# staple/spark-agd

Measured on NVIDIA H100. Metric: AGD examples/sec (rows x applySmooth passes / s), logistic 10M x 1024 dense fp32, higher is better.
Workload: dtype f64

## Files before the change

spark-agd_b200/csrc/k1_tc.cu:

```cuda
#include <cuda.h>
#include <cuda_bf16.h>
#include <cuda_runtime.h>
#include <stdint.h>

#include "agd_common.cuh"
#include "k1_device.cuh"

namespace agd {

namespace {

constexpr int kKR = 16;
constexpr int kRegsConsumer = 64, kRegsAux = 56, kRegsMma = 168;
constexpr int kBlockBytes = kKR * 128;
constexpr int kBBytes = 1024;
constexpr int kScaleOff = 768;

__device__ __forceinline__ uint32_t smem_u32(const void *p) { return (uint32_t)__cvta_generic_to_shared(p); }
__device__ __forceinline__ void mbar_init(uint32_t bar, uint32_t count) {
  asm volatile("mbarrier.init.shared::cta.b64 [%0], %1;" ::"r"(bar), "r"(count));
}
__device__ __forceinline__ void mbar_expect_tx(uint32_t bar, uint32_t bytes) {
  asm volatile("mbarrier.arrive.expect_tx.shared::cta.b64 _, [%0], %1;" ::"r"(bar), "r"(bytes) : "memory");
}
__device__ __forceinline__ void mbar_arrive(uint32_t bar) {
  asm volatile("mbarrier.arrive.shared::cta.b64 _, [%0];" ::"r"(bar) : "memory");
}
__device__ __forceinline__ void mbar_wait(uint32_t bar, uint32_t parity) {
  asm volatile(
      "{\n\t.reg .pred p;\n\t"
      "WAIT_LOOP:\n\t"
      "mbarrier.try_wait.parity.shared::cta.b64 p, [%0], %1;\n\t"
      "@p bra WAIT_DONE;\n\t"
      "bra WAIT_LOOP;\n\t"
      "WAIT_DONE:\n\t}" ::"r"(bar),
      "r"(parity)
      : "memory");
}
__device__ __forceinline__ void named_arrive(int id, int count) {
  asm volatile("bar.arrive %0, %1;" ::"r"(id), "r"(count) : "memory");
}
__device__ __forceinline__ void named_sync(int id, int count) {
  asm volatile("bar.sync %0, %1;" ::"r"(id), "r"(count) : "memory");
}
__device__ __forceinline__ void tma_bulk_g2s(uint32_t dst, const void *src, uint32_t bytes, uint32_t bar) {
  asm volatile("cp.async.bulk.shared::cluster.global.mbarrier::complete_tx::bytes [%0], [%1], %2, [%3];" ::"r"(dst),
               "l"(src), "r"(bytes), "r"(bar)
               : "memory");
}
__device__ __forceinline__ void tma_tile_2d(uint32_t dst, const CUtensorMap *map, int c0, int c1, uint32_t bar) {
  asm volatile("cp.async.bulk.tensor.2d.shared::cluster.global.mbarrier::complete_tx::bytes [%0], [%1, {%2, %3}], [%4];" ::"r"(dst),
               "l"(map), "r"(c0), "r"(c1), "r"(bar)
               : "memory");
}
__device__ __forceinline__ void tma_tile_3d(uint32_t dst, const CUtensorMap *map, int c0, int c1, int c2, uint32_t bar) {
  asm volatile("cp.async.bulk.tensor.3d.shared::cluster.global.mbarrier::complete_tx::bytes [%0], [%1, {%2, %3, %4}], [%5];" ::"r"(dst),
               "l"(map), "r"(c0), "r"(c1), "r"(c2), "r"(bar)
               : "memory");
}
__device__ __forceinline__ uint64_t gmma_desc(uint32_t addr, uint32_t lbo, uint32_t sbo, uint64_t layout) {
  return (uint64_t)((addr & 0x3FFFF) >> 4) | ((uint64_t)(lbo >> 4) << 16) | ((uint64_t)(sbo >> 4) << 32) | (layout << 62);
}
__device__ __forceinline__ void wgmma_fence() { asm volatile("wgmma.fence.sync.aligned;" ::: "memory"); }
__device__ __forceinline__ void wgmma_commit() { asm volatile("wgmma.commit_group.sync.aligned;" ::: "memory"); }
template <int N>
__device__ __forceinline__ void wgmma_wait() { asm volatile("wgmma.wait_group.sync.aligned %0;" ::"n"(N) : "memory"); }
template <int N>
__device__ __forceinline__ void wgmma_bf16(float (&d)[N / 2], uint64_t adesc, uint64_t bdesc);
template <>
__device__ __forceinline__ void wgmma_bf16<16>(float (&d)[8], uint64_t adesc, uint64_t bdesc) {
  asm volatile("{ .reg .pred p; setp.ne.b32 p, 0, 0;\n\t"
               "wgmma.mma_async.sync.aligned.m64n16k16.f32.bf16.bf16 {%0,%1,%2,%3,%4,%5,%6,%7}, %8, %9, p, 1, 1, 1, 0; }"
               : "+f"(d[0]), "+f"(d[1]), "+f"(d[2]), "+f"(d[3]), "+f"(d[4]), "+f"(d[5]), "+f"(d[6]), "+f"(d[7])
               : "l"(adesc), "l"(bdesc)
               : "memory");
}
template <>
__device__ __forceinline__ void wgmma_bf16<24>(float (&d)[12], uint64_t adesc, uint64_t bdesc) {
  asm volatile("{ .reg .pred p; setp.ne.b32 p, 0, 0;\n\t"
               "wgmma.mma_async.sync.aligned.m64n24k16.f32.bf16.bf16 {%0,%1,%2,%3,%4,%5,%6,%7,%8,%9,%10,%11}, %12, %13, p, 1, 1, 1, 0; }"
               : "+f"(d[0]), "+f"(d[1]), "+f"(d[2]), "+f"(d[3]), "+f"(d[4]), "+f"(d[5]), "+f"(d[6]), "+f"(d[7]),
                 "+f"(d[8]), "+f"(d[9]), "+f"(d[10]), "+f"(d[11])
               : "l"(adesc), "l"(bdesc)
               : "memory");
}

template <int N, bool TWO>
__device__ __forceinline__ void mma_accumulate(const float (&e)[2][N / 2], int hb, int hs, const double (&sc)[2], double &g,
                                               double *g2) {
  float v[6];
#pragma unroll
  for (int t = 0; t < (TWO ? 6 : 3); ++t) {
    const int i = t == 0 ? 0 : t == 1 ? 1 : t == 2 ? 4 : t == 3 ? 5 : t == 4 ? 8 : 9;
    const float x0 = hs ? e[0][i + 2] : e[0][i], x1 = hs ? e[1][i + 2] : e[1][i];
    v[t] = hb ? x1 : x0;
  }
  g += (((double)v[0] + (double)v[1]) + (double)v[2]) * sc[0];
  if (TWO) *g2 += (((double)v[3] + (double)v[4]) + (double)v[5]) * sc[1];
}
__device__ __forceinline__ double pow2i(int k) { return __longlong_as_double((long long)(k + 1023) << 52); }
__device__ __forceinline__ void mma_release(uint32_t empty_bar, int lane) {
  __syncwarp();
  if (lane == 0) mbar_arrive(empty_bar);
}

struct TcLayout {
  uint32_t ring_off, w_off, b2_off, partial_off, bars_off, g2_off, total;
};
__host__ __device__ inline TcLayout tc_layout(int ring_groups, int group_bytes, int d, bool two_gradient) {
  TcLayout L;
  L.ring_off = 0;
  L.w_off = (uint32_t)ring_groups * group_bytes;
  L.b2_off = L.w_off + (uint32_t)d * 8;
  L.partial_off = L.b2_off + 2 * kBBytes;
  L.bars_off = L.partial_off + 2 * kKR * 16 * 8;
  L.g2_off = L.bars_off + (2 * (uint32_t)ring_groups + 8) * 8;
  L.total = L.g2_off + (two_gradient ? (uint32_t)d * 8 : 0u);
  return L;
}

struct TcArgs {
  const double *labels;
  const double *w;
  const double *w2;
  double *slabs;
  long long rows;
  int d, kind, slab_stride;
  unsigned long long sample_seed, sample_thresh;
  long long row_base;
  int gb;
  int ngt;
  int ring_groups;
  int one_copy;
  int diag;
};

__host__ __device__ constexpr int tc_consumers(int rpt) { return rpt == 4 ? 256 : 512; }
__device__ __forceinline__ unsigned long long ffma2(unsigned long long a, unsigned long long b, unsigned long long c) {
  const float x = __fmaf_rn(__uint_as_float((uint32_t)a), __uint_as_float((uint32_t)b), __uint_as_float((uint32_t)c));
  const float y = __fmaf_rn(__uint_as_float((uint32_t)(a >> 32)), __uint_as_float((uint32_t)(b >> 32)),
                            __uint_as_float((uint32_t)(c >> 32)));
  return ((unsigned long long)__float_as_uint(y) << 32) | __float_as_uint(x);
}
__device__ __forceinline__ unsigned long long pack2(uint32_t lo, uint32_t hi) {
  unsigned long long d;
  asm("mov.b64 %0, {%1, %2};" : "=l"(d) : "r"(lo), "r"(hi));
  return d;
}

template <int RPT, bool F32, int DUAL = 0>
__global__ void __launch_bounds__(tc_consumers(RPT) + 256, 1)
k1_tc_kernel(const __grid_constant__ CUtensorMap tmap, const __grid_constant__ CUtensorMap tmap3, const TcArgs a,
             const long long ntiles) {
  constexpr int kConsumers = tc_consumers(RPT);
  constexpr int kThreads = kConsumers + 256;
  constexpr int kN = DUAL == 2 ? 24 : 16;
  constexpr int kCW = kConsumers / 32;
  constexpr bool kRepartition = RPT != 4;
  extern __shared__ __align__(1024) unsigned char smem[];
  const int group_bytes = a.gb * kBlockBytes;
  const TcLayout L = tc_layout(a.ring_groups, group_bytes, a.d, DUAL == 2);
  double *w_s = reinterpret_cast<double *>(smem + L.w_off);
  unsigned char *b2 = smem + L.b2_off;
  double *partial = reinterpret_cast<double *>(smem + L.partial_off);
  const uint32_t bars = smem_u32(smem + L.bars_off);
  const int RG = a.ring_groups;
  const uint32_t wbar = bars + 16u * RG, b2_full = wbar + 8, b2_empty = b2_full + 16;
  const int tid = threadIdx.x, warp = tid >> 5, lane = tid & 31;
  const long long my_tiles = (ntiles - blockIdx.x + gridDim.x - 1) / gridDim.x;
  const int npairs = a.d / 128;
  double *slab = a.slabs + (size_t)blockIdx.x * a.slab_stride;

  if (tid == 0) {
    for (int g = 0; g < RG; ++g) {
      mbar_init(bars + 8u * g, 1);
      mbar_init(bars + 8u * (RG + g), 4);
    }
    mbar_init(wbar, 1);
    mbar_init(b2_full, 1); mbar_init(b2_full + 8, 1);
    mbar_init(b2_empty, 4); mbar_init(b2_empty + 8, 4);
    asm volatile("fence.mbarrier_init.release.cluster;" ::: "memory");
  }
  for (int i = tid; i < 2 * kBBytes / 4; i += kThreads) reinterpret_cast<uint32_t *>(b2)[i] = 0u;
  asm volatile("fence.proxy.async.shared::cta;" ::: "memory");
  __syncthreads();

  if (warp >= kCW && warp < kCW + 4) {
   if (kRepartition) asm volatile("setmaxnreg.dec.sync.aligned.u32 %0;" ::"n"(kRegsAux));
   if (warp == kCW) {
    if (lane == 0) {
      mbar_expect_tx(wbar, (uint32_t)a.d * 8u);
      tma_bulk_g2s(smem_u32(w_s), a.w, (uint32_t)a.d * 8u, wbar);
      int slot = -1;
      uint32_t epar = 0;
      bool wrapped = false;
      for (long long k = 0; k < my_tiles; ++k) {
        const long long row0 = (blockIdx.x + k * (long long)gridDim.x) * kKR;
        for (int gi = 0; gi < a.ngt; ++gi) {
          if (++slot == RG) { slot = 0; if (wrapped) epar ^= 1u; wrapped = true; }
          if (wrapped) mbar_wait(bars + 8u * (RG + slot), epar);
          const uint32_t full = bars + 8u * slot;
          mbar_expect_tx(full, (uint32_t)group_bytes);
          if (a.one_copy) {
            tma_tile_3d(smem_u32(smem + (size_t)slot * group_bytes), &tmap3, 0, (int)row0, gi * a.gb, full);
          } else {
            for (int b = 0; b < a.gb; ++b)
              tma_tile_2d(smem_u32(smem + (size_t)slot * group_bytes + b * kBlockBytes), &tmap, (gi * a.gb + b) * 64, (int)row0, full);
          }
        }
      }
    }
   } else if (warp == kCW + 2) {
    double lossacc = 0.0, cntacc = 0.0;
    double ynext = 0.0;
    const int srow = lane & 15;
    const bool second = DUAL && lane >= kKR;
    if (lane < kKR || DUAL) {
      const long long r = (long long)blockIdx.x * kKR + srow;
      if (r < a.rows) ynext = a.labels[r];
    }
    const double *partial2 = partial + 2 * kKR * 2;
    for (long long k = 0; k < my_tiles; ++k) {
      const int bb = (int)(k & 1);
      const long long tile = blockIdx.x + k * (long long)gridDim.x;
      const long long left = a.rows - tile * kKR;
      const int rv = left < kKR ? (int)left : kKR;
      const double ylab = ynext;
      if (lane < kKR || DUAL) {
        const long long r = (tile + gridDim.x) * kKR + srow;
        if (r < a.rows) ynext = a.labels[r];
      }
      named_sync(1 + bb, kConsumers + 32);
      double mult = 0.0;
      bool nonfinite = false;
      if (lane < kKR || second) {
        double m;
        if (RPT) {
          const double *pp = second ? partial2 : partial;
          m = pp[(bb * kKR + srow) * 2] + pp[(bb * kKR + srow) * 2 + 1];
        } else {
          const double *pp = partial + (bb * kKR + lane) * 16;
          m = (((pp[0] + pp[1]) + (pp[2] + pp[3])) + ((pp[4] + pp[5]) + (pp[6] + pp[7]))) +
              (((pp[8] + pp[9]) + (pp[10] + pp[11])) + ((pp[12] + pp[13]) + (pp[14] + pp[15])));
        }
        nonfinite = (lane < kKR || DUAL == 2) && srow < rv && !isfinite(m);
        double mu, loss;
        loss_eval(a.kind, m, ylab, mu, loss);
        if (srow < rv && row_selected(a.sample_seed, a.sample_thresh, a.row_base + tile * kKR + srow)) {
          mult = mu; lossacc += loss; cntacc += 1.0;
        }
      }
      named_arrive(3 + bb, kConsumers + 32);
      const uint32_t hw = (uint32_t)__double2hiint(mult) & 0x7fffffffu;
      const uint32_t hwf = hw | (nonfinite ? 0x80000000u : 0u);
      uint32_t top = __reduce_max_sync(0xffffffffu, lane < kKR ? hwf : 0u), top2 = 0u;
      if (DUAL == 2) top2 = __reduce_max_sync(0xffffffffu, lane < kKR ? 0u : hwf);
      if ((top | top2) >> 31) {
        top = __reduce_max_sync(0xffffffffu, lane < kKR ? hw : 0u);
        if (DUAL == 2) top2 = __reduce_max_sync(0xffffffffu, lane < kKR ? 0u : hw);
        const uint32_t fl = __ballot_sync(0xffffffffu, nonfinite && mult == 0.0);
        const uint32_t zero_rows = DUAL == 2 ? (fl & (fl >> 16) & 0xffffu) : fl;
        const int slot0 = (int)((k * a.ngt) % RG);
#pragma unroll 1
        for (uint32_t rows = zero_rows; rows; rows &= rows - 1u) {
          const int zr = __ffs(rows) - 1;
          int sl = slot0;
#pragma unroll 1
          for (int gi = 0; gi < a.ngt; ++gi) {
#pragma unroll 1
            for (int c = lane; c < a.gb * 8; c += 32)
              *reinterpret_cast<uint4 *>(smem + sl * group_bytes + (c >> 3) * kBlockBytes + zr * 128 + (c & 7) * 16) =
                  make_uint4(0u, 0u, 0u, 0u);
            if (++sl == RG) sl = 0;
          }
        }
      }
      uint32_t E = top >> 20;
      if (DUAL == 2 && second) E = top2 >> 20;
      const int s = E == 0x7ffu ? 0 : E == 0u ? -1022 : E == 0x7feu ? 1023 : (int)E - 1022;
      const int ns = -s;
      const double ms = (mult * pow2i(ns >> 1)) * pow2i(ns - (ns >> 1));
      if (k >= 2) mbar_wait(b2_empty + 8u * bb, (uint32_t)(((k >> 1) - 1) & 1));
      if (srow == 0 && (lane < kKR || (DUAL == 2 && second))) {
        reinterpret_cast<double *>(b2 + bb * kBBytes + kScaleOff)[second ? 1 : 0] = pow2i(s);
      }
      if (lane < kKR || (DUAL == 2 && second)) {
        const __nv_bfloat16 hi = __double2bfloat16(ms);
        const double r1 = ms - (double)__bfloat162float(hi);
        const __nv_bfloat16 mid = __double2bfloat16(r1);
        const double r2 = r1 - (double)__bfloat162float(mid);
        const __nv_bfloat16 lo = __double2bfloat16(r2);
        const int n0 = second ? 9 : 0, n1 = second ? 16 : 1, n2 = second ? 17 : 8;
        unsigned char *base = b2 + bb * kBBytes + (srow / 8) * 128 + (srow % 8) * 2;
#pragma unroll
        for (int t = 0; t < 4; ++t) {
          const int c0 = n0 + 2 * t, c1 = n1 + 2 * t, c2 = n2 + 2 * t;
          *reinterpret_cast<__nv_bfloat16 *>(base + (c0 / 8) * 256 + (c0 % 8) * 16) = hi;
          *reinterpret_cast<__nv_bfloat16 *>(base + (c1 / 8) * 256 + (c1 % 8) * 16) = mid;
          *reinterpret_cast<__nv_bfloat16 *>(base + (c2 / 8) * 256 + (c2 % 8) * 16) = lo;
        }
      }
      asm volatile("fence.proxy.async.shared::cta;" ::: "memory");
      __syncwarp();
      if (lane == 0) mbar_arrive(b2_full + 8u * bb);
    }
    for (int off = DUAL ? 8 : 16; off >= 1; off >>= 1) {
      lossacc += __shfl_xor_sync(0xffffffffu, lossacc, off);
      cntacc += __shfl_xor_sync(0xffffffffu, cntacc, off);
    }
    if (lane == 0) { slab[a.d] = lossacc; slab[a.d + 1] = cntacc; if (!DUAL) { slab[a.d + 2] = 0.0; slab[a.d + 3] = 0.0; } }
    if (DUAL && lane == kKR) {
      slab[a.d + 2] = lossacc; slab[a.d + 3] = cntacc;
      if (DUAL == 2) {
        double *slab2 = slab + a.d + 4;
        slab2[a.d] = lossacc; slab2[a.d + 1] = cntacc; slab2[a.d + 2] = 0.0; slab2[a.d + 3] = 0.0;
      }
    }
   }
  } else if (warp >= kCW + 4) {
    if (kRepartition) asm volatile("setmaxnreg.inc.sync.aligned.u32 %0;" ::"n"(kRegsMma));
    const int mw = warp - (kCW + 4);
    const int q = lane >> 2, j = lane & 3;
    const int hb = j >> 1, hs = j & 1;
    const int fo = 64 * hb + 16 * mw + q + 8 * hs;
    double gacc[32];
#pragma unroll
    for (int p = 0; p < 32; ++p) gacc[p] = 0.0;
    double *g2 = reinterpret_cast<double *>(smem + L.g2_off);
    if (DUAL == 2)
      for (int p = 0; p < npairs; ++p) g2[128 * p + fo] = 0.0;
    const int hp = a.gb / 2;
    int slot = -1;
    uint32_t par = 1;
    float acc[2][kN / 2];
    for (long long k = 0; k < my_tiles; ++k) {
      const int bb = (int)(k & 1);
      mbar_wait(b2_full + 8u * bb, (uint32_t)((k >> 1) & 1));
      const uint64_t bdesc = gmma_desc(smem_u32(b2 + bb * kBBytes), 128, 256, 0);
      const double *scs = reinterpret_cast<const double *>(b2 + bb * kBBytes + kScaleOff);
      const double sc[2] = {scs[0], DUAL == 2 ? scs[1] : 1.0};
#pragma unroll
      for (int p = 0; p < 32; ++p) {
        if (p < npairs) {
          const int pg = p % hp;
          if (pg == 0) {
            if (++slot == RG) slot = 0;
            if (slot == 0) par ^= 1u;
            mbar_wait(bars + 8u * slot, par);
          }
          const uint32_t a0 = smem_u32(smem + (size_t)slot * group_bytes + (2 * pg) * kBlockBytes);
          wgmma_fence();
          if (a.diag != 101) {
            wgmma_bf16<kN>(acc[0], gmma_desc(a0, kBlockBytes, 1024, 1), bdesc);
            wgmma_bf16<kN>(acc[1], gmma_desc(a0 + kBlockBytes, kBlockBytes, 1024, 1), bdesc);
          }
          wgmma_commit();
          wgmma_wait<0>();
          mma_accumulate<kN, DUAL == 2>(acc, hb, hs, sc, gacc[p], g2 + 128 * p + fo);
          if (pg == hp - 1) mma_release(bars + 8u * (RG + slot), lane);
        }
      }
      __syncwarp();
      if (lane == 0) mbar_arrive(b2_empty + 8u * bb);
    }
#pragma unroll
    for (int p = 0; p < 32; ++p)
      if (p < npairs) {
        slab[128 * p + fo] = gacc[p];
        if (DUAL == 2) slab[a.d + 4 + 128 * p + fo] = g2[128 * p + fo];
      }
  } else {
    if (kRepartition) asm volatile("setmaxnreg.dec.sync.aligned.u32 %0;" ::"n"(kRegsConsumer));
    if constexpr (RPT == 0) {
      const int r = lane & 15, hsel = lane >> 4;
      mbar_wait(wbar, 0);
      int slot = -1;
      uint32_t par = 1;
      const int npairs = a.gb * 4;
      uint32_t x_off[2];
      int w_off[2];
      bool act[2];
#pragma unroll
      for (int j = 0; j < 2; ++j) {
        const int c = 2 * (warp + 16 * j) + hsel;
        act[j] = warp + 16 * j < npairs;
        x_off[j] = (uint32_t)((c >> 3) * kBlockBytes + r * 128 + (((c & 7) ^ (r & 7)) << 4));
        w_off[j] = c * 8;
      }
      for (long long k = 0; k < my_tiles; ++k) {
        const int bb = (int)(k & 1);
        double pa[2] = {0.0, 0.0}, pb[2] = {0.0, 0.0};
        const double *wp = w_s;
        for (int gi = 0; gi < a.ngt; ++gi) {
          if (++slot == RG) slot = 0;
          if (slot == 0) par ^= 1u;
          mbar_wait(bars + 8u * slot, par);
          if (a.diag != 100) {
            const unsigned char *gbase = smem + (uint32_t)slot * (uint32_t)group_bytes;
#pragma unroll
            for (int j = 0; j < 2; ++j) {
              if (act[j]) {
                const uint4 xr = *reinterpret_cast<const uint4 *>(gbase + x_off[j]);
                const double2 *wv = reinterpret_cast<const double2 *>(wp + w_off[j]);
#pragma unroll
                for (int q = 0; q < 4; ++q) {
                  const double2 wq = wv[q];
                  const uint32_t xw = q == 0 ? xr.x : q == 1 ? xr.y : q == 2 ? xr.z : xr.w;
                  pa[j] = fma((double)__uint_as_float(xw << 16), wq.x, pa[j]);
                  pb[j] = fma((double)__uint_as_float(xw & 0xffff0000u), wq.y, pb[j]);
                }
              }
            }
          }
          wp += a.gb * 64;
        }
        double p = (pa[0] + pb[0]) + (pa[1] + pb[1]);
        p += __shfl_xor_sync(0xffffffffu, p, 16);
        if (k >= 2) named_sync(3 + bb, kConsumers + 32);
        if (lane < 16) partial[(bb * kKR + r) * 16 + warp] = p;
        named_arrive(1 + bb, kConsumers + 32);
      }
    } else {
    constexpr int kSlots = kKR / (RPT ? RPT : 1);
    const int rq = tid >> 6;
    const int vv = tid & 63;
    mbar_wait(wbar, 0);
    int slot = -1;
    uint32_t par = 1;
    const int blk = vv >> 3, ch = vv & 7;
    const bool active = vv < a.gb * 8;
    uint32_t x_off[RPT];
#pragma unroll
    for (int j = 0; j < RPT; ++j) {
      const int row = rq + j * kSlots;
      x_off[j] = (uint32_t)(blk * kBlockBytes + row * 128 + ((ch ^ (row & 7)) << 4));
    }
    if constexpr (F32) {
      const int nchunks = a.d / 8;
      float4 lo4[2], hi4[2], lo4b[2], hi4b[2];
#pragma unroll
      for (int i = 0; i < 2; ++i) {
        const int c = tid + i * kConsumers;
        if (c < nchunks) {
          const double *src = w_s + (size_t)c * 8;
          lo4[i] = make_float4((float)src[0], (float)src[1], (float)src[2], (float)src[3]);
          hi4[i] = make_float4((float)src[4], (float)src[5], (float)src[6], (float)src[7]);
          if (DUAL) {
            const double *s2 = a.w2 + (size_t)c * 8;
            lo4b[i] = make_float4((float)s2[0], (float)s2[1], (float)s2[2], (float)s2[3]);
            hi4b[i] = make_float4((float)s2[4], (float)s2[5], (float)s2[6], (float)s2[7]);
          }
        }
      }
      named_sync(5, kConsumers);
      float4 *plane0 = reinterpret_cast<float4 *>(w_s), *plane1 = plane0 + nchunks;
      float4 *plane0b = plane1 + nchunks, *plane1b = plane0b + nchunks;
#pragma unroll
      for (int i = 0; i < 2; ++i) {
        const int c = tid + i * kConsumers;
        if (c < nchunks) {
          plane0[c] = lo4[i]; plane1[c] = hi4[i];
          if (DUAL) { plane0b[c] = lo4b[i]; plane1b[c] = hi4b[i]; }
        }
      }
      named_sync(5, kConsumers);
      double *partial2 = partial + 2 * kKR * 2;
      for (long long k = 0; k < my_tiles; ++k) {
        const int bb = (int)(k & 1);
        double pd[RPT], pd2[RPT];
        unsigned long long acc[RPT], acc2[RPT];
#pragma unroll
        for (int j = 0; j < RPT; ++j) { pd[j] = 0.0; acc[j] = 0ull; pd2[j] = 0.0; acc2[j] = 0ull; }
        const ulonglong2 *wp0 = reinterpret_cast<const ulonglong2 *>(plane0) + vv;
        const ulonglong2 *wp1 = reinterpret_cast<const ulonglong2 *>(plane1) + vv;
        const ulonglong2 *wq0 = reinterpret_cast<const ulonglong2 *>(plane0b) + vv;
        const ulonglong2 *wq1 = reinterpret_cast<const ulonglong2 *>(plane1b) + vv;
        for (int gi = 0; gi < a.ngt; ++gi) {
          if (++slot == RG) slot = 0;
          if (slot == 0) par ^= 1u;
          mbar_wait(bars + 8u * slot, par);
          if (active && a.diag != 100) {
            const unsigned char *gbase = smem + (uint32_t)slot * (uint32_t)group_bytes;
            uint4 xr[RPT];
#pragma unroll
            for (int j = 0; j < RPT; ++j) xr[j] = *reinterpret_cast<const uint4 *>(gbase + x_off[j]);
            const ulonglong2 wa = *wp0, wb = *wp1;
            ulonglong2 va = wa, vb = wb;
            if (DUAL) { va = *wq0; vb = *wq1; }
#pragma unroll
            for (int j = 0; j < RPT; ++j) {
              const unsigned long long x0 = pack2(xr[j].x << 16, xr[j].x & 0xffff0000u), x1 = pack2(xr[j].y << 16, xr[j].y & 0xffff0000u),
                                       x2 = pack2(xr[j].z << 16, xr[j].z & 0xffff0000u), x3 = pack2(xr[j].w << 16, xr[j].w & 0xffff0000u);
              acc[j] = ffma2(x0, wa.x, acc[j]);
              acc[j] = ffma2(x1, wa.y, acc[j]);
              acc[j] = ffma2(x2, wb.x, acc[j]);
              acc[j] = ffma2(x3, wb.y, acc[j]);
              if (DUAL) {
                acc2[j] = ffma2(x0, va.x, acc2[j]);
                acc2[j] = ffma2(x1, va.y, acc2[j]);
                acc2[j] = ffma2(x2, vb.x, acc2[j]);
                acc2[j] = ffma2(x3, vb.y, acc2[j]);
              }
            }
          }
          wp0 += a.gb * 8;
          wp1 += a.gb * 8;
          wq0 += a.gb * 8;
          wq1 += a.gb * 8;
          if ((gi & 1) || gi + 1 == a.ngt) {
#pragma unroll
            for (int j = 0; j < RPT; ++j) {
              pd[j] += (double)(__uint_as_float((uint32_t)acc[j]) + __uint_as_float((uint32_t)(acc[j] >> 32)));
              acc[j] = 0ull;
              if (DUAL) {
                pd2[j] += (double)(__uint_as_float((uint32_t)acc2[j]) + __uint_as_float((uint32_t)(acc2[j] >> 32)));
                acc2[j] = 0ull;
              }
            }
          }
        }
        const double tot = warp_rows_reduce<RPT>(pd, lane);
        double tot2 = 0.0;
        if (DUAL) tot2 = warp_rows_reduce<RPT>(pd2, lane);
        if (k >= 2) named_sync(3 + bb, kConsumers + 32);
        if ((lane & (32 / RPT - 1)) == 0) {
          partial[(bb * kKR + rq + kSlots * (lane / (32 / RPT))) * 2 + (warp & 1)] = tot;
          if (DUAL) partial2[(bb * kKR + rq + kSlots * (lane / (32 / RPT))) * 2 + (warp & 1)] = tot2;
        }
        named_arrive(1 + bb, kConsumers + 32);
      }
    } else {
    for (int c = tid; c < a.d / 8; c += kConsumers) {
      const int f = (c >> 1) & 3;
      if (f) {
        double2 *blk = reinterpret_cast<double2 *>(w_s + (size_t)c * 8);
        const double2 t0 = blk[0], t1 = blk[1], t2 = blk[2], t3 = blk[3];
        const double2 v[4] = {t0, t1, t2, t3};
        blk[0 ^ f] = v[0]; blk[1 ^ f] = v[1]; blk[2 ^ f] = v[2]; blk[3 ^ f] = v[3];
      }
    }
    named_sync(5, kConsumers);
    const int sw = (lane >> 1) & 3;
    for (long long k = 0; k < my_tiles; ++k) {
      const int bb = (int)(k & 1);
      double pa[RPT], pb[RPT];
#pragma unroll
      for (int j = 0; j < RPT; ++j) { pa[j] = 0.0; pb[j] = 0.0; }
      const double *wp = w_s + (blk * 64 + ch * 8);
      for (int gi = 0; gi < a.ngt; ++gi) {
        if (++slot == RG) slot = 0;
        if (slot == 0) par ^= 1u;
        mbar_wait(bars + 8u * slot, par);
        if (active && a.diag != 100) {
          const unsigned char *gbase = smem + (uint32_t)slot * (uint32_t)group_bytes;
          uint4 xr[RPT];
#pragma unroll
          for (int j = 0; j < RPT; ++j) xr[j] = *reinterpret_cast<const uint4 *>(gbase + x_off[j]);
#pragma unroll
          for (int q = 0; q < 4; ++q) {
            const double2 wq = *reinterpret_cast<const double2 *>(wp + 2 * (q ^ sw));
#pragma unroll
            for (int j = 0; j < RPT; ++j) {
              const uint32_t xw = q == 0 ? xr[j].x : q == 1 ? xr[j].y : q == 2 ? xr[j].z : xr[j].w;
              pa[j] = fma((double)__uint_as_float(xw << 16), wq.x, pa[j]);
              pb[j] = fma((double)__uint_as_float(xw & 0xffff0000u), wq.y, pb[j]);
            }
          }
        }
        wp += a.gb * 64;
      }
      double p[RPT];
#pragma unroll
      for (int j = 0; j < RPT; ++j) p[j] = pa[j] + pb[j];
      const double tot = warp_rows_reduce<RPT>(p, lane);
      if (k >= 2) named_sync(3 + bb, kConsumers + 32);
      if ((lane & (32 / RPT - 1)) == 0) partial[(bb * kKR + rq + kSlots * (lane / (32 / RPT))) * 2 + (warp & 1)] = tot;
      named_arrive(1 + bb, kConsumers + 32);
    }
    }
    }
  }
}

template <int SITE, typename K>
cudaError_t set_smem_once(K kern, int bytes) {
  static int cur[64] = {0};
  int dev = 0;
  cudaError_t e = cudaGetDevice(&dev);
  if (e != cudaSuccess) return e;
  if (dev >= 0 && dev < 64 && cur[dev] == bytes) return cudaSuccess;
  e = cudaFuncSetAttribute(kern, cudaFuncAttributeMaxDynamicSharedMemorySize, bytes);
  if (e == cudaSuccess && dev >= 0 && dev < 64) cur[dev] = bytes;
  return e;
}

typedef CUresult (*EncodeTiledFn)(CUtensorMap *, CUtensorMapDataType, cuuint32_t, void *, const cuuint64_t *, const cuuint64_t *,
                                  const cuuint32_t *, const cuuint32_t *, CUtensorMapInterleave, CUtensorMapSwizzle,
                                  CUtensorMapL2promotion, CUtensorMapFloatOOBfill);

}

int k1_tc_supported(int32_t d, int elem_bytes) { return elem_bytes == 2 && d >= 128 && d <= 4096 && d % 128 == 0; }

cudaError_t k1_tc_launch(const K1Args &a, int sm_count, int *blocks_out, cudaStream_t st) {
  if (!k1_tc_supported(a.d, 2)) return cudaErrorInvalidValue;
  if (a.rows <= 0) { *blocks_out = 0; return cudaSuccess; }
  static EncodeTiledFn encode = nullptr;
  if (!encode) {
    void *fn = nullptr;
    cudaDriverEntryPointQueryResult qres;
    cudaError_t e = cudaGetDriverEntryPoint("cuTensorMapEncodeTiled", &fn, cudaEnableDefault, &qres);
    if (e != cudaSuccess || !fn) return e != cudaSuccess ? e : cudaErrorUnknown;
    encode = (EncodeTiledFn)fn;
  }
  CUtensorMap tmap;
  const cuuint64_t gdim[2] = {(cuuint64_t)a.d, (cuuint64_t)a.rows};
  const cuuint64_t gstr[1] = {(cuuint64_t)a.d * 2};
  const cuuint32_t box[2] = {64, (cuuint32_t)kKR};
  const cuuint32_t estr[2] = {1, 1};
  if (encode(&tmap, CU_TENSOR_MAP_DATA_TYPE_BFLOAT16, 2, const_cast<void *>(a.X), gdim, gstr, box, estr,
             CU_TENSOR_MAP_INTERLEAVE_NONE, CU_TENSOR_MAP_SWIZZLE_128B, CU_TENSOR_MAP_L2_PROMOTION_L2_256B,
             CU_TENSOR_MAP_FLOAT_OOB_FILL_NONE) != CUDA_SUCCESS)
    return cudaErrorInvalidValue;
  const int nblk = a.d / 64;
  int gb = 8;
  while (nblk % gb) gb -= 2;
  CUtensorMap tmap3;
  {
    const cuuint64_t gdim3[3] = {64, (cuuint64_t)a.rows, (cuuint64_t)nblk};
    const cuuint64_t gstr3[2] = {(cuuint64_t)a.d * 2, 128};
    const cuuint32_t box3[3] = {64, (cuuint32_t)kKR, (cuuint32_t)gb};
    const cuuint32_t estr3[3] = {1, 1, 1};
    if (encode(&tmap3, CU_TENSOR_MAP_DATA_TYPE_BFLOAT16, 3, const_cast<void *>(a.X), gdim3, gstr3, box3, estr3,
               CU_TENSOR_MAP_INTERLEAVE_NONE, CU_TENSOR_MAP_SWIZZLE_128B, CU_TENSOR_MAP_L2_PROMOTION_L2_256B,
               CU_TENSOR_MAP_FLOAT_OOB_FILL_NONE) != CUDA_SUCCESS)
      return cudaErrorInvalidValue;
  }
  TcArgs t;
  t.one_copy = a.tune_ctas == 2 ? 0 : 1;
  t.diag = (a.kind == 100 || a.kind == 101) ? a.kind : 0;
  if (a.w2 && (a.tune_rows != 0 || a.tc_margins_f64)) return cudaErrorInvalidValue;
  t.labels = a.labels; t.w = a.w; t.w2 = a.w2; t.slabs = a.slabs; t.rows = a.rows; t.d = a.d; t.kind = a.kind;
  t.slab_stride = a.slab_stride;
  t.sample_seed = a.sample_seed; t.sample_thresh = a.sample_thresh; t.row_base = a.row_base;
  t.gb = gb;
  t.ngt = nblk / gb;
  const int group_bytes = t.gb * kBlockBytes;
  int ring = a.stages > 0 ? a.stages : 16;
  const bool two_gradient = a.w2 && a.dual_full;
  const uint32_t budget = 227u * 1024u - 2048u;
  while (ring > 2 && tc_layout(ring, group_bytes, a.d, two_gradient).total + 1024 > budget) --ring;
  if (ring < t.ngt + 1) ring = t.ngt + 1;
  t.ring_groups = ring;
  const TcLayout L = tc_layout(ring, group_bytes, a.d, two_gradient);
  if (L.total + 1024 > budget) return cudaErrorInvalidValue;
  const long long ntiles = (a.rows + kKR - 1) / kKR;
  long long grid = sm_count;
  if (grid > ntiles) grid = ntiles;
  *blocks_out = (int)grid;
  const int smem_bytes = (int)L.total + 1024;
  cudaError_t e;
  if (a.tune_rows == 1) {
    e = set_smem_once<1>(k1_tc_kernel<0, false, 0>, smem_bytes);
    if (e != cudaSuccess) return e;
    k1_tc_kernel<0, false, 0><<<(unsigned)grid, 768, smem_bytes, st>>>(tmap, tmap3, t, ntiles);
  } else if (a.tune_rows == 4) {
    e = set_smem_once<2>(k1_tc_kernel<4, false, 0>, smem_bytes);
    if (e != cudaSuccess) return e;
    k1_tc_kernel<4, false, 0><<<(unsigned)grid, 512, smem_bytes, st>>>(tmap, tmap3, t, ntiles);
  } else if (a.tc_margins_f64) {
    e = set_smem_once<3>(k1_tc_kernel<2, false, 0>, smem_bytes);
    if (e != cudaSuccess) return e;
    k1_tc_kernel<2, false, 0><<<(unsigned)grid, 768, smem_bytes, st>>>(tmap, tmap3, t, ntiles);
  } else if (a.w2 && a.dual_full) {
    e = set_smem_once<6>(k1_tc_kernel<2, true, 2>, smem_bytes);
    if (e != cudaSuccess) return e;
    k1_tc_kernel<2, true, 2><<<(unsigned)grid, 768, smem_bytes, st>>>(tmap, tmap3, t, ntiles);
  } else if (a.w2) {
    e = set_smem_once<4>(k1_tc_kernel<2, true, 1>, smem_bytes);
    if (e != cudaSuccess) return e;
    k1_tc_kernel<2, true, 1><<<(unsigned)grid, 768, smem_bytes, st>>>(tmap, tmap3, t, ntiles);
  } else {
    e = set_smem_once<5>(k1_tc_kernel<2, true, 0>, smem_bytes);
    if (e != cudaSuccess) return e;
    k1_tc_kernel<2, true, 0><<<(unsigned)grid, 768, smem_bytes, st>>>(tmap, tmap3, t, ntiles);
  }
  return cudaGetLastError();
}

}
```

Baseline: 1.031 billion.

## Double-buffer wgmma accumulators in MMA warps with shared-memory gradient accumulation

Adds a path for the MMA warps that keeps the gradient accumulators in shared memory rather than a 32-entry register array. This frees registers for two sets of wgmma accumulators, so the next pair's wgmma can be issued before the previous one is retired (wait<1> instead of wait<0>). The path is chosen only when it leaves the smem ring deep enough. The cost is extra shared-memory traffic on every accumulate and possibly a smaller TMA ring.

After: 1.029 billion, median of 6. No clear change (-0.2%).

```diff
diff --git a/spark-agd_b200/csrc/k1_tc.cu b/spark-agd_b200/csrc/k1_tc.cu
--- a/spark-agd_b200/csrc/k1_tc.cu
+++ b/spark-agd_b200/csrc/k1_tc.cu
@@ -105,17 +105,17 @@
 }
 
 struct TcLayout {
-  uint32_t ring_off, w_off, b2_off, partial_off, bars_off, g2_off, total;
+  uint32_t ring_off, w_off, b2_off, partial_off, bars_off, g_off, total;
 };
-__host__ __device__ inline TcLayout tc_layout(int ring_groups, int group_bytes, int d, bool two_gradient) {
+__host__ __device__ inline TcLayout tc_layout(int ring_groups, int group_bytes, int d, bool g_smem) {
   TcLayout L;
   L.ring_off = 0;
   L.w_off = (uint32_t)ring_groups * group_bytes;
   L.b2_off = L.w_off + (uint32_t)d * 8;
   L.partial_off = L.b2_off + 2 * kBBytes;
   L.bars_off = L.partial_off + 2 * kKR * 16 * 8;
-  L.g2_off = L.bars_off + (2 * (uint32_t)ring_groups + 8) * 8;
-  L.total = L.g2_off + (two_gradient ? (uint32_t)d * 8 : 0u);
+  L.g_off = L.bars_off + (2 * (uint32_t)ring_groups + 8) * 8;
+  L.total = L.g_off + (g_smem ? (uint32_t)d * 8 : 0u);
   return L;
 }
 
@@ -133,6 +133,7 @@
   int ring_groups;
   int one_copy;
   int diag;
+  int g_smem;
 };
 
 __host__ __device__ constexpr int tc_consumers(int rpt) { return rpt == 4 ? 256 : 512; }
@@ -159,7 +160,7 @@
   constexpr bool kRepartition = RPT != 4;
   extern __shared__ __align__(1024) unsigned char smem[];
   const int group_bytes = a.gb * kBlockBytes;
-  const TcLayout L = tc_layout(a.ring_groups, group_bytes, a.d, DUAL == 2);
+  const TcLayout L = tc_layout(a.ring_groups, group_bytes, a.d, DUAL == 2 || a.g_smem);
   double *w_s = reinterpret_cast<double *>(smem + L.w_off);
   unsigned char *b2 = smem + L.b2_off;
   double *partial = reinterpret_cast<double *>(smem + L.partial_off);
@@ -323,15 +324,63 @@
     const int q = lane >> 2, j = lane & 3;
     const int hb = j >> 1, hs = j & 1;
     const int fo = 64 * hb + 16 * mw + q + 8 * hs;
-    double gacc[32];
-#pragma unroll
-    for (int p = 0; p < 32; ++p) gacc[p] = 0.0;
-    double *g2 = reinterpret_cast<double *>(smem + L.g2_off);
-    if (DUAL == 2)
-      for (int p = 0; p < npairs; ++p) g2[128 * p + fo] = 0.0;
+    double *gs = reinterpret_cast<double *>(smem + L.g_off);
+    if (DUAL == 2 || a.g_smem)
+      for (int p = 0; p < npairs; ++p) gs[128 * p + fo] = 0.0;
     const int hp = a.gb / 2;
     int slot = -1;
     uint32_t par = 1;
+    if (DUAL != 2 && a.g_smem) {
+    float acc[2][2][kN / 2];
+    int ps[2];
+    for (long long k = 0; k < my_tiles; ++k) {
+      const int bb = (int)(k & 1);
+      mbar_wait(b2_full + 8u * bb, (uint32_t)((k >> 1) & 1));
+      const uint64_t bdesc = gmma_desc(smem_u32(b2 + bb * kBBytes), 128, 256, 0);
+      const double sc[2] = {reinterpret_cast<const double *>(b2 + bb * kBBytes + kScaleOff)[0], 1.0};
+      auto issue = [&](const int p, float (&e)[2][kN / 2], int &pslot) {
+        const int pg = p % hp;
+        if (pg == 0) {
+          if (++slot == RG) slot = 0;
+          if (slot == 0) par ^= 1u;
+          mbar_wait(bars + 8u * slot, par);
+        }
+        pslot = slot;
+        const uint32_t a0 = smem_u32(smem + (size_t)slot * group_bytes + (2 * pg) * kBlockBytes);
+        wgmma_fence();
+        if (a.diag != 101) {
+          wgmma_bf16<kN>(e[0], gmma_desc(a0, kBlockBytes, 1024, 1), bdesc);
+          wgmma_bf16<kN>(e[1], gmma_desc(a0 + kBlockBytes, kBlockBytes, 1024, 1), bdesc);
+        }
+      };
+      auto retire = [&](const int p, const float (&e)[2][kN / 2], const int pslot) {
+        mma_accumulate<kN, false>(e, hb, hs, sc, gs[128 * p + fo], nullptr);
+        if (p % hp == hp - 1) mma_release(bars + 8u * (RG + pslot), lane);
+      };
+      issue(0, acc[0], ps[0]);
+      wgmma_commit();
+#pragma unroll 1
+      for (int p = 0; p < npairs; p += 2) {
+        if (p + 1 < npairs) issue(p + 1, acc[1], ps[1]);
+        wgmma_commit();
+        wgmma_wait<1>();
+        retire(p, acc[0], ps[0]);
+        if (p + 1 < npairs) {
+          if (p + 2 < npairs) issue(p + 2, acc[0], ps[0]);
+          wgmma_commit();
+          wgmma_wait<1>();
+          retire(p + 1, acc[1], ps[1]);
+        }
+      }
+      wgmma_wait<0>();
+      __syncwarp();
+      if (lane == 0) mbar_arrive(b2_empty + 8u * bb);
+    }
+    for (int p = 0; p < npairs; ++p) slab[128 * p + fo] = gs[128 * p + fo];
+    } else {
+    double gacc[32];
+#pragma unroll
+    for (int p = 0; p < 32; ++p) gacc[p] = 0.0;
     float acc[2][kN / 2];
     for (long long k = 0; k < my_tiles; ++k) {
       const int bb = (int)(k & 1);
@@ -356,7 +405,7 @@
           }
           wgmma_commit();
           wgmma_wait<0>();
-          mma_accumulate<kN, DUAL == 2>(acc, hb, hs, sc, gacc[p], g2 + 128 * p + fo);
+          mma_accumulate<kN, DUAL == 2>(acc, hb, hs, sc, gacc[p], gs + 128 * p + fo);
           if (pg == hp - 1) mma_release(bars + 8u * (RG + slot), lane);
         }
       }
@@ -367,8 +416,9 @@
     for (int p = 0; p < 32; ++p)
       if (p < npairs) {
         slab[128 * p + fo] = gacc[p];
-        if (DUAL == 2) slab[a.d + 4 + 128 * p + fo] = g2[128 * p + fo];
-      }
+        if (DUAL == 2) slab[a.d + 4 + 128 * p + fo] = gs[128 * p + fo];
+      }
+    }
   } else {
     if (kRepartition) asm volatile("setmaxnreg.dec.sync.aligned.u32 %0;" ::"n"(kRegsConsumer));
     if constexpr (RPT == 0) {
@@ -647,12 +697,19 @@
   t.ngt = nblk / gb;
   const int group_bytes = t.gb * kBlockBytes;
   int ring = a.stages > 0 ? a.stages : 16;
+  const uint32_t budget = 227u * 1024u - 2048u;
   const bool two_gradient = a.w2 && a.dual_full;
-  const uint32_t budget = 227u * 1024u - 2048u;
-  while (ring > 2 && tc_layout(ring, group_bytes, a.d, two_gradient).total + 1024 > budget) --ring;
-  if (ring < t.ngt + 1) ring = t.ngt + 1;
+  auto ring_for = [&](bool g_smem) {
+    int r = ring;
+    while (r > 2 && tc_layout(r, group_bytes, a.d, g_smem).total + 1024 > budget) --r;
+    return r < t.ngt + 1 ? t.ngt + 1 : r;
+  };
+  const int ring_reg = ring_for(two_gradient);
+  const int ring_smem = ring_for(true);
+  t.g_smem = !two_gradient && ring_smem >= (ring_reg < t.ngt + 3 ? ring_reg : t.ngt + 3);
+  ring = t.g_smem ? ring_smem : ring_reg;
   t.ring_groups = ring;
-  const TcLayout L = tc_layout(ring, group_bytes, a.d, two_gradient);
+  const TcLayout L = tc_layout(ring, group_bytes, a.d, two_gradient || t.g_smem);
   if (L.total + 1024 > budget) return cudaErrorInvalidValue;
   const long long ntiles = (a.rows + kKR - 1) / kKR;
   long long grid = sm_count;
```
